# lucasjinreal/yolov7_d2

Measured on AMD Instinct MI355X. Metric: images/sec training, YOLOX-s 640x640 bs=16/GPU, higher is better.
Workload: dtype bf16; 1 GPU; YOLOX-s CSPDarknet+PAFPN 640x640 bs=16/GPU: fwd + SimOTA loss + bwd + grad all-reduce + SGD(momentum) step, uint8 image batch + labels resident in HBM; global_batch=16, parallelism=dp1, hipgraph=True

## Files before the change

### yolov7_d2_amd/csrc/misc_ops.hip

```cpp
#include <stdlib.h>
#include "common.h"

static int ew_blocks(int64_t total, int cap = 4096) {
  int64_t b = (total + 255) / 256;
  if (b > cap) b = cap;
  if (b < 1) b = 1;
  return (int)b;
}

__global__ __launch_bounds__(256) void focus_pack_kernel(const float* __restrict__ img, int N, int H, int W,
                                                         __bf16* out, int ldo) {
  const int Ho = H / 2, Wo = W / 2;
  const int64_t total = (int64_t)N * Ho * Wo;
  for (int64_t idx = blockIdx.x * 256LL + threadIdx.x; idx < total; idx += (int64_t)gridDim.x * 256) {
    const int ox = (int)(idx % Wo);
    const int64_t r = idx / Wo;
    const int oy = (int)(r % Ho), n = (int)(r / Ho);
    float f[16];
#pragma unroll
    for (int q = 0; q < 4; ++q) {
      const int dy = q & 1, dx = q >> 1;
#pragma unroll
      for (int c = 0; c < 3; ++c)
        f[q * 3 + c] = img[(((int64_t)n * 3 + c) * H + (2 * oy + dy)) * W + 2 * ox + dx];
// ... 297 lines not shown
extern "C" int mi_maxpool3x3s2_fwd(const void* x, int ldx, void* y, int ldy, int N, int H, int W, int C, mi_stream_t st) {
  MI_REQUIRE(x && y && C % 8 == 0 && ldx % 8 == 0 && ldy % 8 == 0 && N > 0 && H > 0 && W > 0, "maxpool3x3s2_fwd: args");
  const int64_t total = (int64_t)N * ((H + 1) / 2) * ((W + 1) / 2) * (C / 8);
  hipLaunchKernelGGL(maxpool3x3s2_fwd_kernel, dim3(ew_blocks(total)), dim3(256), 0, (hipStream_t)st, (const __bf16*)x,
                     ldx, (__bf16*)y, ldy, N, H, W, C / 8);
  MI_CHECK_LAUNCH("maxpool3x3s2_fwd");
  return MI_OK;
}
extern "C" int mi_maxpool3x3s2_bwd(const void* x, int ldx, const void* dy, int lddy, void* dx, int lddx, int accumulate,
                                   int N, int H, int W, int C, mi_stream_t st) {
  MI_REQUIRE(x && dy && dx && C % 8 == 0 && ldx % 8 == 0 && lddy % 8 == 0 && lddx % 8 == 0, "maxpool3x3s2_bwd: args");
  const int64_t total = (int64_t)N * H * W * (C / 8);
  hipLaunchKernelGGL(maxpool3x3s2_bwd_kernel, dim3(ew_blocks(total)), dim3(256), 0, (hipStream_t)st, (const __bf16*)x,
                     ldx, (const __bf16*)dy, lddy, (__bf16*)dx, lddx, accumulate, N, H, W, C / 8);
  MI_CHECK_LAUNCH("maxpool3x3s2_bwd");
  return MI_OK;
}

__global__ __launch_bounds__(256) void upsample2x_fwd_kernel(const __bf16* __restrict__ x, int ldx, __bf16* y, int ldy,
                                                             int N, int H, int W, int C8) {
  const int Ho = 2 * H, Wo = 2 * W;
  const int64_t total = (int64_t)N * Ho * Wo * C8;
  for (int64_t idx = blockIdx.x * 256LL + threadIdx.x; idx < total; idx += (int64_t)gridDim.x * 256) {
    const int c8 = (int)(idx % C8);
    int64_t r = idx / C8;
    const int ox = (int)(r % Wo); r /= Wo;
    const int oy = (int)(r % Ho);
    const int n = (int)(r / Ho);
    const bf16x8 v = *(const bf16x8*)(x + (((int64_t)n * H + oy / 2) * W + ox / 2) * ldx + c8 * 8);
    *(bf16x8*)(y + (((int64_t)n * Ho + oy) * Wo + ox) * ldy + c8 * 8) = v;
  }
}
__global__ __launch_bounds__(256) void upsample2x_bwd_kernel(const __bf16* __restrict__ dy, int lddy, __bf16* dx,
                                                             int lddx, int accumulate, int N, int H, int W, int C8) {
  const int Ho = 2 * H, Wo = 2 * W;
  const int64_t total = (int64_t)N * H * W * C8;
  for (int64_t idx = blockIdx.x * 256LL + threadIdx.x; idx < total; idx += (int64_t)gridDim.x * 256) {
    const int c8 = (int)(idx % C8);
    int64_t r = idx / C8;
    const int ix = (int)(r % W); r /= W;
    const int iy = (int)(r % H);
    const int n = (int)(r / H);
    float acc[8];
#pragma unroll
    for (int e = 0; e < 8; ++e) acc[e] = 0.f;
#pragma unroll
    for (int a = 0; a < 2; ++a)
#pragma unroll
      for (int b = 0; b < 2; ++b) {
        const bf16x8 v = *(const bf16x8*)(dy + (((int64_t)n * Ho + 2 * iy + a) * Wo + 2 * ix + b) * lddy + c8 * 8);
#pragma unroll
        for (int e = 0; e < 8; ++e) acc[e] += (float)v[e];
      }
    __bf16* dp = dx + (((int64_t)n * H + iy) * W + ix) * lddx + c8 * 8;
    if (accumulate) {
      const bf16x8 o = *(const bf16x8*)dp;
#pragma unroll
      for (int e = 0; e < 8; ++e) acc[e] += (float)o[e];
    }
    *(bf16x8*)dp = pack8(acc);
  }
}

extern "C" int mi_upsample2x_fwd(const void* x, int ldx, void* y, int ldy, int N, int H, int W, int C,
                                 mi_stream_t st) {
  MI_REQUIRE(x && y && C % 8 == 0 && ldx % 8 == 0 && ldy % 8 == 0, "upsample_fwd: args");
  const int64_t total = (int64_t)N * 4 * H * W * (C / 8);
  hipLaunchKernelGGL(upsample2x_fwd_kernel, dim3(ew_blocks(total)), dim3(256), 0, (hipStream_t)st, (const __bf16*)x,
                     ldx, (__bf16*)y, ldy, N, H, W, C / 8);
  MI_CHECK_LAUNCH("upsample_fwd");
  return MI_OK;
}
extern "C" int mi_upsample2x_bwd(const void* dy, int lddy, void* dx, int lddx, int accumulate, int N, int H, int W,
                                 int C, mi_stream_t st) {
  MI_REQUIRE(dy && dx && C % 8 == 0 && lddy % 8 == 0 && lddx % 8 == 0, "upsample_bwd: args");
  const int64_t total = (int64_t)N * H * W * (C / 8);
  hipLaunchKernelGGL(upsample2x_bwd_kernel, dim3(ew_blocks(total)), dim3(256), 0, (hipStream_t)st, (const __bf16*)dy,
                     lddy, (__bf16*)dx, lddx, accumulate, N, H, W, C / 8);
  MI_CHECK_LAUNCH("upsample_bwd");
  return MI_OK;
}

#define SPP_T 512
__global__ __launch_bounds__(SPP_T) void spp_fwd_plane_kernel(const __bf16* __restrict__ x, int ldx, __bf16* y5,
                                                            __bf16* y9, __bf16* y13, int ldy, uint8_t* idx, int N,
                                                            int H, int W, int C8) {
  extern __shared__ __attribute__((aligned(16))) char smem[];
  const int HW = H * W, C = C8 * 8;
  bf16x8* Xp = (bf16x8*)smem;
  bf16x8* Hv = Xp + HW;
  uint64_t* Hc = (uint64_t*)(Hv + HW);
  const int lb = (gridDim.x % 8 == 0) ? (int)(blockIdx.x % 8) * (int)(gridDim.x / 8) + (int)(blockIdx.x / 8) : (int)blockIdx.x;
  const int c8 = lb % C8, n = lb / C8;
  const int64_t npix = (int64_t)N * HW;
  const __bf16* xb = x + ((int64_t)n * HW) * ldx + c8 * 8;
  for (int p = threadIdx.x; p < HW; p += SPP_T) Xp[p] = *(const bf16x8*)(xb + (int64_t)p * ldx);
  __syncthreads();
  const int k = blockIdx.y, r = 2 + 2 * k;
  for (int p = threadIdx.x; p < HW; p += SPP_T) {
    const int py = p / W, px = p - py * W;
    float m[8];
    uint8_t am[8];
#pragma unroll
    for (int e = 0; e < 8; ++e) { m[e] = -INFINITY; am[e] = 6; }
    for (int dx = -r; dx <= r; ++dx) {
      const int xx = px + dx;
      if (xx < 0 || xx >= W) continue;
      const bf16x8 v = Xp[py * W + xx];
#pragma unroll
      for (int e = 0; e < 8; ++e) {
        const float f = (float)v[e];
        if (f > m[e]) { m[e] = f; am[e] = (uint8_t)(dx + 6); }
      }
    }
    Hv[p] = pack8(m);
    uint64_t pk = 0;
#pragma unroll
    for (int e = 0; e < 8; ++e) pk |= (uint64_t)am[e] << (8 * e);
    Hc[p] = pk;
    *(uint64_t*)(idx + ((int64_t)(3 + k) * npix + (int64_t)n * HW + p) * C + c8 * 8) = pk;
  }
  __syncthreads();
  __bf16* yk = k == 0 ? y5 : (k == 1 ? y9 : y13);
  for (int p = threadIdx.x; p < HW; p += SPP_T) {
    const int py = p / W, px = p - py * W;
    float m[8];
    uint8_t am[8];
#pragma unroll
    for (int e = 0; e < 8; ++e) { m[e] = -INFINITY; am[e] = 6; }
    for (int dy = -r; dy <= r; ++dy) {
      const int yy = py + dy;
      if (yy < 0 || yy >= H) continue;
      const bf16x8 v = Hv[yy * W + px];
#pragma unroll
      for (int e = 0; e < 8; ++e) {
        const float f = (float)v[e];
        if (f > m[e]) { m[e] = f; am[e] = (uint8_t)(dy + 6); }
      }
    }
    const int64_t pix = (int64_t)n * HW + p;
    *(bf16x8*)(yk + pix * ldy + c8 * 8) = pack8(m);
    uint64_t pk = 0;
#pragma unroll
    for (int e = 0; e < 8; ++e) pk |= (uint64_t)am[e] << (8 * e);
    *(uint64_t*)(idx + ((int64_t)k * npix + pix) * C + c8 * 8) = pk;
  }
}

__global__ __launch_bounds__(SPP_T) void spp_bwd_plane_kernel(const __bf16* __restrict__ d5, const __bf16* __restrict__ d9,
                                                            const __bf16* __restrict__ d13, int lddy,
                                                            const uint8_t* __restrict__ idx, __bf16* dx, int lddx,
                                                            int accumulate, int N, int H, int W, int C8) {
  extern __shared__ __attribute__((aligned(16))) char smem[];
  const int HW = H * W, C = C8 * 8;
  bf16x8* Gp = (bf16x8*)smem;
  uint64_t* Dy = (uint64_t*)(Gp + HW);
  uint64_t* Dx = Dy + HW;
  float* Gh = (float*)(Dx + HW);
  const int lb = (gridDim.x % 8 == 0) ? (int)(blockIdx.x % 8) * (int)(gridDim.x / 8) + (int)(blockIdx.x / 8) : (int)blockIdx.x;
  const int c8 = lb % C8, n = lb / C8;
  const int64_t npix = (int64_t)N * HW;
  float acc[2][8];
  for (int i = 0; i < 2; ++i)
#pragma unroll
    for (int e = 0; e < 8; ++e) acc[i][e] = 0.f;
  for (int k = 0; k < 3; ++k) {
    const int r = 2 + 2 * k;
    const __bf16* dk = k == 0 ? d5 : (k == 1 ? d9 : d13);
    __syncthreads();
    for (int p = threadIdx.x; p < HW; p += SPP_T) {
      const int64_t pix = (int64_t)n * HW + p;
      Gp[p] = *(const bf16x8*)(dk + pix * lddy + c8 * 8);
      Dy[p] = *(const uint64_t*)(idx + ((int64_t)k * npix + pix) * C + c8 * 8);
      Dx[p] = *(const uint64_t*)(idx + ((int64_t)(3 + k) * npix + pix) * C + c8 * 8);
    }
    __syncthreads();
    for (int q = threadIdx.x; q < HW; q += SPP_T) {
      const int qy = q / W, qx = q - qy * W;
      float g[8];
#pragma unroll
      for (int e = 0; e < 8; ++e) g[e] = 0.f;
      for (int dy = -r; dy <= r; ++dy) {
        const int oy = qy - dy;
        if (oy < 0 || oy >= H) continue;
        const int o = oy * W + qx;
        const uint64_t pk = Dy[o];
        const bf16x8 gv = Gp[o];
        const uint8_t code = (uint8_t)(dy + 6);
#pragma unroll
        for (int e = 0; e < 8; ++e)
          if ((uint8_t)(pk >> (8 * e)) == code) g[e] += (float)gv[e];
      }
#pragma unroll
      for (int e = 0; e < 8; ++e) Gh[q * 8 + e] = g[e];
    }
    __syncthreads();
#pragma unroll
    for (int i = 0; i < 2; ++i) {
      const int p = threadIdx.x + i * SPP_T;
      if (p >= HW) continue;
      const int py = p / W, px = p - py * W;
      for (int dxx = -r; dxx <= r; ++dxx) {
        const int qx = px - dxx;
        if (qx < 0 || qx >= W) continue;
        const int q = py * W + qx;
        const uint64_t pk = Dx[q];
        const uint8_t code = (uint8_t)(dxx + 6);
#pragma unroll
        for (int e = 0; e < 8; ++e)
          if ((uint8_t)(pk >> (8 * e)) == code) acc[i][e] += Gh[q * 8 + e];
      }
    }
  }
#pragma unroll
  for (int i = 0; i < 2; ++i) {
    const int p = threadIdx.x + i * SPP_T;
    if (p >= HW) continue;
    __bf16* op_ = dx + ((int64_t)n * HW + p) * lddx + c8 * 8;
    float o[8];
#pragma unroll
    for (int e = 0; e < 8; ++e) o[e] = acc[i][e];
    if (accumulate) {
      const bf16x8 ov = *(const bf16x8*)op_;
#pragma unroll
      for (int e = 0; e < 8; ++e) o[e] += (float)ov[e];
    }
    *(bf16x8*)op_ = pack8(o);
  }
}

extern "C" int mi_spp_pool_fwd(const void* x, int ldx, void* y5, void* y9, void* y13, int ldy, uint8_t* idx, int N,
                               int H, int W, int C, mi_stream_t st) {
  MI_REQUIRE(x && y5 && y9 && y13 && idx && C % 8 == 0 && ldx % 8 == 0 && ldy % 8 == 0, "spp_fwd: args");
  const size_t lds = (size_t)H * W * 40;
  MI_REQUIRE(lds <= 160 * 1024, "spp_fwd: plane %dx%d too large for the LDS kernel", H, W);
  static bool attr_done = false;
  if (!attr_done) {
    hipFuncSetAttribute((const void*)spp_fwd_plane_kernel, hipFuncAttributeMaxDynamicSharedMemorySize, 160 * 1024);
    hipFuncSetAttribute((const void*)spp_bwd_plane_kernel, hipFuncAttributeMaxDynamicSharedMemorySize, 160 * 1024);
    attr_done = true;
  }
  hipLaunchKernelGGL(spp_fwd_plane_kernel, dim3(N * (C / 8), 3), dim3(SPP_T), lds, (hipStream_t)st, (const __bf16*)x, ldx,
                     (__bf16*)y5, (__bf16*)y9, (__bf16*)y13, ldy, idx, N, H, W, C / 8);
  MI_CHECK_LAUNCH("spp_fwd");
  return MI_OK;
}
extern "C" int mi_spp_pool_bwd(const void* dy5, const void* dy9, const void* dy13, int lddy, const uint8_t* idx,
                               void* dx, int lddx, int accumulate, int N, int H, int W, int C, mi_stream_t st) {
  MI_REQUIRE(dy5 && dy9 && dy13 && idx && dx && C % 8 == 0 && lddy % 8 == 0 && lddx % 8 == 0, "spp_bwd: args");
  MI_REQUIRE(H * W <= 2 * SPP_T, "spp_bwd: plane %dx%d > %d pixels (register accumulators)", H, W, 2 * SPP_T);
  const size_t lds = (size_t)H * W * 64;
  static bool attr_done = false;
  if (!attr_done) {
    hipFuncSetAttribute((const void*)spp_fwd_plane_kernel, hipFuncAttributeMaxDynamicSharedMemorySize, 160 * 1024);
    hipFuncSetAttribute((const void*)spp_bwd_plane_kernel, hipFuncAttributeMaxDynamicSharedMemorySize, 160 * 1024);
    attr_done = true;
  }
  hipLaunchKernelGGL(spp_bwd_plane_kernel, dim3(N * (C / 8)), dim3(SPP_T), lds, (hipStream_t)st, (const __bf16*)dy5,
                     (const __bf16*)dy9, (const __bf16*)dy13, lddy, idx, (__bf16*)dx, lddx, accumulate, N, H, W, C / 8);
  MI_CHECK_LAUNCH("spp_bwd");
  return MI_OK;
}

__global__ __launch_bounds__(256) void copy_bf16_kernel(const __bf16* __restrict__ src, int lds_, __bf16* dst, int ldd,
                                                        int accumulate, int64_t npix, int C8) {
  const int64_t total = npix * C8;
  for (int64_t idx = blockIdx.x * 256LL + threadIdx.x; idx < total; idx += (int64_t)gridDim.x * 256) {
    const int64_t pix = idx / C8;
    const int c8 = (int)(idx - pix * C8);
    const bf16x8 v = *(const bf16x8*)(src + pix * lds_ + c8 * 8);
    __bf16* dp = dst + pix * ldd + c8 * 8;
    if (accumulate) {
      const bf16x8 o = *(const bf16x8*)dp;
      float f[8];
#pragma unroll
      for (int e = 0; e < 8; ++e) f[e] = (float)o[e] + (float)v[e];
      *(bf16x8*)dp = pack8(f);
    } else {
      *(bf16x8*)dp = v;
    }
  }
}
extern "C" int mi_copy_bf16(const void* src, int lds_, void* dst, int ldd, int accumulate, int64_t npix, int C,
                            mi_stream_t st) {
  MI_REQUIRE(src && dst && C % 8 == 0 && lds_ % 8 == 0 && ldd % 8 == 0, "copy_bf16: args");
  hipLaunchKernelGGL(copy_bf16_kernel, dim3(ew_blocks(npix * (C / 8))), dim3(256), 0, (hipStream_t)st,
                     (const __bf16*)src, lds_, (__bf16*)dst, ldd, accumulate, npix, C / 8);
  MI_CHECK_LAUNCH("copy_bf16");
  return MI_OK;
}

__global__ __launch_bounds__(256) void colsum_stage1_kernel(const __bf16* __restrict__ x, int ldx, int64_t npix,
                                                            int C8N, float* __restrict__ part) {
  __shared__ float red[256 * 8];
  const int tid = threadIdx.x;
  const int c8 = tid % C8N, pl = tid / C8N, PL = 256 / C8N;
  float s[8];
#pragma unroll
  for (int e = 0; e < 8; ++e) s[e] = 0.f;
  if (pl < PL)
    for (int64_t p = (int64_t)blockIdx.x * PL + pl; p < npix; p += (int64_t)gridDim.x * PL) {
      const bf16x8 v = *(const bf16x8*)(x + p * ldx + c8 * 8);
#pragma unroll
      for (int e = 0; e < 8; ++e) s[e] += (float)v[e];
    }
#pragma unroll
  for (int e = 0; e < 8; ++e) red[tid * 8 + e] = (pl < PL) ? s[e] : 0.f;
  __syncthreads();
  const int C = C8N * 8;
  if (tid < C) {
    const int cc8 = tid >> 3, e = tid & 7;
    float a = 0.f;
    for (int q = 0; q < PL; ++q) a += red[(q * C8N + cc8) * 8 + e];
    part[(size_t)blockIdx.x * C + tid] = a;
  }
}
__global__ __launch_bounds__(128) void colsum_stage2_kernel(const float* __restrict__ part, int nblk, int CP, int C,
                                                            float* out, int accumulate) {
  const int c = threadIdx.x;
  if (c >= C) return;
  float a = 0.f;
  for (int b = 0; b < nblk; ++b) a += part[(size_t)b * CP + c];
  out[c] = accumulate ? out[c] + a : a;
}
extern "C" int mi_colsum_bf16(const void* x, int ldx, int64_t npix, int C, float* out, int accumulate, float* ws,
                              mi_stream_t st) {
  MI_REQUIRE(x && out && ws && C > 0 && C <= 128, "colsum: C %d (<=128)", C);
  const int CP = (C + 7) / 8 * 8;
  const int C8N = CP / 8;
  MI_REQUIRE(ldx % 8 == 0 && ((uintptr_t)x % 16) == 0 && ldx >= CP, "colsum: alignment / ld");
  hipStream_t s = (hipStream_t)st;
  const int PL = 256 / C8N;
  int nblk = (int)((npix + PL * 8 - 1) / (PL * 8));
  if (nblk > 128) nblk = 128;
  if (nblk < 1) nblk = 1;
  hipLaunchKernelGGL(colsum_stage1_kernel, dim3(nblk), dim3(256), 0, s, (const __bf16*)x, ldx, npix, C8N, ws);
  MI_CHECK_LAUNCH("colsum1");
  hipLaunchKernelGGL(colsum_stage2_kernel, dim3(1), dim3(128), 0, s, ws, nblk, CP, C, out, accumulate);
  MI_CHECK_LAUNCH("colsum2");
  return MI_OK;
}

// ... 196 lines not shown
```

Measured before the change: 3081 images/sec.

## Compute SPP pools with packed value/position keys and cascaded separable max windows

The SPP forward now packs each bf16 value with its window position into an order-preserving 32-bit key. It then computes the 5/9/13 max pools as a cascade of separable 5-wide passes (SPPF-style) in one block per plane, where before there were three independent direct-window launches. Argmax codes come from the key's position bits. The backward keeps gradients as fp32 in LDS, prefetches the next pool's gradients and codes into registers while the current pool computes, and uses branchless masked adds. This cuts redundant window comparisons and load latency, at the cost of more LDS per pixel and a fallback path for large planes.

```diff
diff --git a/yolov7_d2_amd/csrc/misc_ops.hip b/yolov7_d2_amd/csrc/misc_ops.hip
--- a/yolov7_d2_amd/csrc/misc_ops.hip
+++ b/yolov7_d2_amd/csrc/misc_ops.hip
@@ -403,9 +403,135 @@
 }
 
 #define SPP_T 512
+#define SPP_FWD_LDS_PER_PIXEL 160
+__device__ __forceinline__ uint32_t spp_key(uint32_t b, uint32_t pos8) {
+  const uint32_t nz = b == 0x8000u;
+  const uint32_t img = nz ? 0x8000u : ((b & 0x8000u) ? (~b & 0xFFFFu) : (b | 0x8000u));
+  return (img - 0x80u <= 0xFF00u) ? (img << 16 | pos8 | nz) : 0u;
+}
+__device__ __forceinline__ uint32_t spp_key_bits(uint32_t key) {
+  const uint32_t img = key >> 16;
+  const uint32_t b = (key & 1u) ? 0x8000u : ((img & 0x8000u) ? (img & 0x7FFFu) : (~img & 0xFFFFu));
+  return img ? b : 0xFF80u;
+}
+struct SppK8 { uint32_t v[8]; };
+__device__ __forceinline__ SppK8 spp_ld(const uint4* m, int HW, int p) {
+  const uint4 a = m[p], b = m[HW + p];
+  return SppK8{{a.x, a.y, a.z, a.w, b.x, b.y, b.z, b.w}};
+}
+__device__ __forceinline__ void spp_st(uint4* m, int HW, int p, const SppK8& k) {
+  m[p] = make_uint4(k.v[0], k.v[1], k.v[2], k.v[3]);
+  m[HW + p] = make_uint4(k.v[4], k.v[5], k.v[6], k.v[7]);
+}
+__device__ __forceinline__ SppK8 spp_max(const SppK8& a, const SppK8& b) {
+  SppK8 r;
+#pragma unroll
+  for (int e = 0; e < 8; ++e) r.v[e] = max(a.v[e], b.v[e]);
+  return r;
+}
+__device__ __forceinline__ SppK8 spp_win5(const uint4* m, int HW, int base, int stride, int c, int n) {
+  SppK8 r = spp_ld(m, HW, base + c * stride);
+#pragma unroll
+  for (int d = -2; d <= 2; ++d)
+    if (d) r = spp_max(r, spp_ld(m, HW, base + min(max(c + d, 0), n - 1) * stride));
+  return r;
+}
+__device__ __forceinline__ SppK8 spp_win9(const uint4* m, int HW, int base, int stride, int c, int n) {
+  return spp_max(spp_ld(m, HW, base + max(c - 2, 0) * stride), spp_ld(m, HW, base + min(c + 2, n - 1) * stride));
+}
+__device__ __forceinline__ SppK8 spp_win13(const uint4* m, int HW, int base, int stride, int c, int n) {
+  return spp_max(spp_ld(m, HW, base + c * stride), spp_max(spp_ld(m, HW, base + max(c - 4, 0) * stride),
+                                                           spp_ld(m, HW, base + min(c + 4, n - 1) * stride)));
+}
+__device__ __forceinline__ uint64_t spp_codes(const SppK8& k, uint32_t cb) {
+  uint64_t pk = 0;
+#pragma unroll
+  for (int e = 0; e < 8; ++e) pk |= (uint64_t)((k.v[e] >> 16) ? cb - ((k.v[e] >> 8) & 0xFFu) : 6u) << (8 * e);
+  return pk;
+}
+__device__ __forceinline__ uint4 spp_values(const SppK8& k) {
+  uint32_t w[4];
+#pragma unroll
+  for (int e = 0; e < 4; ++e) w[e] = spp_key_bits(k.v[2 * e]) | spp_key_bits(k.v[2 * e + 1]) << 16;
+  return make_uint4(w[0], w[1], w[2], w[3]);
+}
+__device__ __forceinline__ SppK8 spp_rekey(const SppK8& k, uint32_t pos8) {
+  SppK8 r;
+#pragma unroll
+  for (int e = 0; e < 8; ++e) r.v[e] = (k.v[e] >> 16) ? ((k.v[e] & 0xFFFF0001u) | pos8) : 0u;
+  return r;
+}
 __global__ __launch_bounds__(SPP_T) void spp_fwd_plane_kernel(const __bf16* __restrict__ x, int ldx, __bf16* y5,
                                                             __bf16* y9, __bf16* y13, int ldy, uint8_t* idx, int N,
                                                             int H, int W, int C8) {
+  extern __shared__ __attribute__((aligned(16))) char smem[];
+  const int HW = H * W, C = C8 * 8;
+  uint4* Kx = (uint4*)smem;
+  uint4* H5 = Kx + 2 * HW;
+  uint4* R9 = H5 + 2 * HW;
+  uint4* R13 = R9 + 2 * HW;
+  uint4* T13 = R13 + 2 * HW;
+  const int lb = (gridDim.x % 8 == 0) ? (int)(blockIdx.x % 8) * (int)(gridDim.x / 8) + (int)(blockIdx.x / 8) : (int)blockIdx.x;
+  const int c8 = lb % C8, n = lb / C8;
+  const int64_t npix = (int64_t)N * HW, pix0 = (int64_t)n * HW;
+  const uint16_t* xb = (const uint16_t*)x + pix0 * ldx + c8 * 8;
+  for (int p = threadIdx.x; p < HW; p += SPP_T) {
+    const uint4 v = *(const uint4*)(xb + (int64_t)p * ldx);
+    const uint32_t pos8 = (uint32_t)(255 - p % W) << 8;
+    const uint32_t w[4] = {v.x, v.y, v.z, v.w};
+    SppK8 k;
+#pragma unroll
+    for (int e = 0; e < 4; ++e) {
+      k.v[2 * e] = spp_key(w[e] & 0xFFFFu, pos8);
+      k.v[2 * e + 1] = spp_key(w[e] >> 16, pos8);
+    }
+    spp_st(Kx, HW, p, k);
+  }
+  __syncthreads();
+  uint8_t* cx = idx + (3 * npix + pix0) * C + c8 * 8;
+  uint8_t* cy = idx + pix0 * C + c8 * 8;
+  for (int p = threadIdx.x; p < HW; p += SPP_T) {
+    const int py = p / W, px = p - py * W;
+    const SppK8 h = spp_win5(Kx, HW, py * W, 1, px, W);
+    spp_st(H5, HW, p, h);
+    *(uint64_t*)(cx + (int64_t)p * C) = spp_codes(h, 261u - px);
+  }
+  __syncthreads();
+  for (int p = threadIdx.x; p < HW; p += SPP_T) {
+    const int py = p / W, px = p - py * W;
+    const uint32_t row8 = (uint32_t)(255 - py) << 8;
+    spp_st(Kx, HW, p, spp_rekey(spp_ld(H5, HW, p), row8));
+    const SppK8 h9 = spp_win9(H5, HW, py * W, 1, px, W);
+    *(uint64_t*)(cx + (npix + p) * C) = spp_codes(h9, 261u - px);
+    spp_st(R9, HW, p, spp_rekey(h9, row8));
+    const SppK8 h13 = spp_win13(H5, HW, py * W, 1, px, W);
+    *(uint64_t*)(cx + (2 * npix + p) * C) = spp_codes(h13, 261u - px);
+    spp_st(R13, HW, p, spp_rekey(h13, row8));
+  }
+  __syncthreads();
+  for (int p = threadIdx.x; p < HW; p += SPP_T) {
+    const int py = p / W, px = p - py * W;
+    const SppK8 v = spp_win5(Kx, HW, px, W, py, H);
+    *(uint4*)(y5 + (pix0 + p) * ldy + c8 * 8) = spp_values(v);
+    *(uint64_t*)(cy + (int64_t)p * C) = spp_codes(v, 261u - py);
+    spp_st(H5, HW, p, spp_win5(R9, HW, px, W, py, H));
+    spp_st(T13, HW, p, spp_win5(R13, HW, px, W, py, H));
+  }
+  __syncthreads();
+  for (int p = threadIdx.x; p < HW; p += SPP_T) {
+    const int py = p / W, px = p - py * W;
+    const SppK8 v9 = spp_win9(H5, HW, px, W, py, H);
+    *(uint4*)(y9 + (pix0 + p) * ldy + c8 * 8) = spp_values(v9);
+    *(uint64_t*)(cy + (npix + p) * C) = spp_codes(v9, 261u - py);
+    const SppK8 v13 = spp_win13(T13, HW, px, W, py, H);
+    *(uint4*)(y13 + (pix0 + p) * ldy + c8 * 8) = spp_values(v13);
+    *(uint64_t*)(cy + (2 * npix + p) * C) = spp_codes(v13, 261u - py);
+  }
+}
+
+static __global__ __launch_bounds__(SPP_T) void spp_fwd_taps_kernel(const __bf16* __restrict__ x, int ldx, __bf16* y5,
+                                                                  __bf16* y9, __bf16* y13, int ldy, uint8_t* idx,
+                                                                  int N, int H, int W, int C8) {
   extern __shared__ __attribute__((aligned(16))) char smem[];
   const int HW = H * W, C = C8 * 8;
   bf16x8* Xp = (bf16x8*)smem;
@@ -468,16 +594,22 @@
   }
 }
 
+__device__ __forceinline__ void spp_add_where(float* acc, uint2 codes, uint32_t code, const float4& a, const float4& b) {
+  const float g[8] = {a.x, a.y, a.z, a.w, b.x, b.y, b.z, b.w};
+#pragma unroll
+  for (int e = 0; e < 8; ++e)
+    acc[e] += (((e < 4 ? codes.x : codes.y) >> (8 * (e & 3))) & 0xFFu) == code ? g[e] : 0.f;
+}
 __global__ __launch_bounds__(SPP_T) void spp_bwd_plane_kernel(const __bf16* __restrict__ d5, const __bf16* __restrict__ d9,
                                                             const __bf16* __restrict__ d13, int lddy,
                                                             const uint8_t* __restrict__ idx, __bf16* dx, int lddx,
                                                             int accumulate, int N, int H, int W, int C8) {
   extern __shared__ __attribute__((aligned(16))) char smem[];
   const int HW = H * W, C = C8 * 8;
-  bf16x8* Gp = (bf16x8*)smem;
-  uint64_t* Dy = (uint64_t*)(Gp + HW);
-  uint64_t* Dx = Dy + HW;
-  float* Gh = (float*)(Dx + HW);
+  float4* Gp = (float4*)smem;
+  float4* Gh = Gp + 2 * HW;
+  uint2* Dy = (uint2*)(Gh + 2 * HW);
+  uint2* Dx = Dy + HW;
   const int lb = (gridDim.x % 8 == 0) ? (int)(blockIdx.x % 8) * (int)(gridDim.x / 8) + (int)(blockIdx.x / 8) : (int)blockIdx.x;
   const int c8 = lb % C8, n = lb / C8;
   const int64_t npix = (int64_t)N * HW;
@@ -485,35 +617,49 @@
   for (int i = 0; i < 2; ++i)
 #pragma unroll
     for (int e = 0; e < 8; ++e) acc[i][e] = 0.f;
+  uint4 ng[2];
+  uint2 ny[2], nx[2];
+  auto fetch = [&](int k) {
+    const __bf16* dk = k == 0 ? d5 : (k == 1 ? d9 : d13);
+#pragma unroll
+    for (int i = 0; i < 2; ++i) {
+      const int p = threadIdx.x + i * SPP_T;
+      if (p >= HW) continue;
+      const int64_t pix = (int64_t)n * HW + p;
+      ng[i] = *(const uint4*)(dk + pix * lddy + c8 * 8);
+      ny[i] = *(const uint2*)(idx + ((int64_t)k * npix + pix) * C + c8 * 8);
+      nx[i] = *(const uint2*)(idx + ((int64_t)(3 + k) * npix + pix) * C + c8 * 8);
+    }
+  };
+  fetch(0);
   for (int k = 0; k < 3; ++k) {
     const int r = 2 + 2 * k;
-    const __bf16* dk = k == 0 ? d5 : (k == 1 ? d9 : d13);
     __syncthreads();
-    for (int p = threadIdx.x; p < HW; p += SPP_T) {
-      const int64_t pix = (int64_t)n * HW + p;
-      Gp[p] = *(const bf16x8*)(dk + pix * lddy + c8 * 8);
-      Dy[p] = *(const uint64_t*)(idx + ((int64_t)k * npix + pix) * C + c8 * 8);
-      Dx[p] = *(const uint64_t*)(idx + ((int64_t)(3 + k) * npix + pix) * C + c8 * 8);
+#pragma unroll
+    for (int i = 0; i < 2; ++i) {
+      const int p = threadIdx.x + i * SPP_T;
+      if (p >= HW) continue;
+      Gp[p] = make_float4(__uint_as_float(ng[i].x << 16), __uint_as_float(ng[i].x & 0xFFFF0000u),
+                          __uint_as_float(ng[i].y << 16), __uint_as_float(ng[i].y & 0xFFFF0000u));
+      Gp[HW + p] = make_float4(__uint_as_float(ng[i].z << 16), __uint_as_float(ng[i].z & 0xFFFF0000u),
+                               __uint_as_float(ng[i].w << 16), __uint_as_float(ng[i].w & 0xFFFF0000u));
+      Dy[p] = ny[i];
+      Dx[p] = nx[i];
     }
     __syncthreads();
+    if (k < 2) fetch(k + 1);
     for (int q = threadIdx.x; q < HW; q += SPP_T) {
       const int qy = q / W, qx = q - qy * W;
       float g[8];
 #pragma unroll
       for (int e = 0; e < 8; ++e) g[e] = 0.f;
-      for (int dy = -r; dy <= r; ++dy) {
-        const int oy = qy - dy;
-        if (oy < 0 || oy >= H) continue;
+      const int o1 = max(qy - r, 0);
+      for (int oy = min(qy + r, H - 1); oy >= o1; --oy) {
         const int o = oy * W + qx;
-        const uint64_t pk = Dy[o];
-        const bf16x8 gv = Gp[o];
-        const uint8_t code = (uint8_t)(dy + 6);
-#pragma unroll
-        for (int e = 0; e < 8; ++e)
-          if ((uint8_t)(pk >> (8 * e)) == code) g[e] += (float)gv[e];
+        spp_add_where(g, Dy[o], (uint32_t)(qy - oy + 6), Gp[o], Gp[HW + o]);
       }
-#pragma unroll
-      for (int e = 0; e < 8; ++e) Gh[q * 8 + e] = g[e];
+      Gh[q] = make_float4(g[0], g[1], g[2], g[3]);
+      Gh[HW + q] = make_float4(g[4], g[5], g[6], g[7]);
     }
     __syncthreads();
 #pragma unroll
@@ -521,15 +667,10 @@
       const int p = threadIdx.x + i * SPP_T;
       if (p >= HW) continue;
       const int py = p / W, px = p - py * W;
-      for (int dxx = -r; dxx <= r; ++dxx) {
-        const int qx = px - dxx;
-        if (qx < 0 || qx >= W) continue;
+      const int q1 = max(px - r, 0);
+      for (int qx = min(px + r, W - 1); qx >= q1; --qx) {
         const int q = py * W + qx;
-        const uint64_t pk = Dx[q];
-        const uint8_t code = (uint8_t)(dxx + 6);
-#pragma unroll
-        for (int e = 0; e < 8; ++e)
-          if ((uint8_t)(pk >> (8 * e)) == code) acc[i][e] += Gh[q * 8 + e];
+        spp_add_where(acc[i], Dx[q], (uint32_t)(px - qx + 6), Gh[q], Gh[HW + q]);
       }
     }
   }
@@ -553,16 +694,22 @@
 extern "C" int mi_spp_pool_fwd(const void* x, int ldx, void* y5, void* y9, void* y13, int ldy, uint8_t* idx, int N,
                                int H, int W, int C, mi_stream_t st) {
   MI_REQUIRE(x && y5 && y9 && y13 && idx && C % 8 == 0 && ldx % 8 == 0 && ldy % 8 == 0, "spp_fwd: args");
-  const size_t lds = (size_t)H * W * 40;
-  MI_REQUIRE(lds <= 160 * 1024, "spp_fwd: plane %dx%d too large for the LDS kernel", H, W);
   static bool attr_done = false;
   if (!attr_done) {
     hipFuncSetAttribute((const void*)spp_fwd_plane_kernel, hipFuncAttributeMaxDynamicSharedMemorySize, 160 * 1024);
-    hipFuncSetAttribute((const void*)spp_bwd_plane_kernel, hipFuncAttributeMaxDynamicSharedMemorySize, 160 * 1024);
+    hipFuncSetAttribute((const void*)spp_fwd_taps_kernel, hipFuncAttributeMaxDynamicSharedMemorySize, 160 * 1024);
     attr_done = true;
   }
-  hipLaunchKernelGGL(spp_fwd_plane_kernel, dim3(N * (C / 8), 3), dim3(SPP_T), lds, (hipStream_t)st, (const __bf16*)x, ldx,
-                     (__bf16*)y5, (__bf16*)y9, (__bf16*)y13, ldy, idx, N, H, W, C / 8);
+  const size_t lds = (size_t)H * W * SPP_FWD_LDS_PER_PIXEL;
+  if (lds <= 160 * 1024 && H <= 256 && W <= 256) {
+    hipLaunchKernelGGL(spp_fwd_plane_kernel, dim3(N * (C / 8)), dim3(SPP_T), lds, (hipStream_t)st, (const __bf16*)x, ldx,
+                       (__bf16*)y5, (__bf16*)y9, (__bf16*)y13, ldy, idx, N, H, W, C / 8);
+  } else {
+    const size_t lds_taps = (size_t)H * W * 40;
+    MI_REQUIRE(lds_taps <= 160 * 1024, "spp_fwd: plane %dx%d too large for the LDS kernel", H, W);
+    hipLaunchKernelGGL(spp_fwd_taps_kernel, dim3(N * (C / 8), 3), dim3(SPP_T), lds_taps, (hipStream_t)st, (const __bf16*)x,
+                       ldx, (__bf16*)y5, (__bf16*)y9, (__bf16*)y13, ldy, idx, N, H, W, C / 8);
+  }
   MI_CHECK_LAUNCH("spp_fwd");
   return MI_OK;
 }
@@ -570,10 +717,9 @@
                                void* dx, int lddx, int accumulate, int N, int H, int W, int C, mi_stream_t st) {
   MI_REQUIRE(dy5 && dy9 && dy13 && idx && dx && C % 8 == 0 && lddy % 8 == 0 && lddx % 8 == 0, "spp_bwd: args");
   MI_REQUIRE(H * W <= 2 * SPP_T, "spp_bwd: plane %dx%d > %d pixels (register accumulators)", H, W, 2 * SPP_T);
-  const size_t lds = (size_t)H * W * 64;
+  const size_t lds = (size_t)H * W * 80;
   static bool attr_done = false;
   if (!attr_done) {
-    hipFuncSetAttribute((const void*)spp_fwd_plane_kernel, hipFuncAttributeMaxDynamicSharedMemorySize, 160 * 1024);
     hipFuncSetAttribute((const void*)spp_bwd_plane_kernel, hipFuncAttributeMaxDynamicSharedMemorySize, 160 * 1024);
     attr_done = true;
   }
```

New measurement: 3098 images/sec, median of 6. No clear change (+0.5%).

## Rewrite SPP pooling kernels with packed-key max and fused kernel sizes

Applied to the files above, without the earlier changes.

The SPP forward max-pool kernel now packs each bf16 value together with its coordinate into a sortable 32-bit key, so argmax becomes a plain integer max. Growing windows (5/9/13) are computed incrementally in a single block when the plane fits in one round. Block size is chosen to match the plane size. The backward kernel preloads all three gradients and indices into registers, replaces branches with clamped, predicated taps, and for small planes processes all three kernel sizes in one pass. This cuts redundant LDS scans, divergent branches and kernel work, at the cost of more LDS and registers per block and extra code complexity.

```diff
diff --git a/yolov7_d2_amd/csrc/misc_ops.hip b/yolov7_d2_amd/csrc/misc_ops.hip
--- a/yolov7_d2_amd/csrc/misc_ops.hip
+++ b/yolov7_d2_amd/csrc/misc_ops.hip
@@ -403,139 +403,254 @@
 }
 
 #define SPP_T 512
+__device__ __forceinline__ uint32_t spp_word(uint32_t b, uint32_t cf) {
+  const uint32_t nz = b == 0x8000u ? 1u : 0u;
+  const uint32_t key = nz ? 0x8000u : (b ^ ((b & 0x8000u) ? 0xFFFFu : 0x8000u));
+  return key << 16 | cf | nz;
+}
+__device__ __forceinline__ uint32_t spp_bits(uint32_t w) {
+  const uint32_t key = w >> 16;
+  return key ^ ((key & 0x8000u) ? 0x8000u : 0xFFFFu) ^ ((w & 1u) << 15);
+}
+__device__ __forceinline__ uint32_t spp_coord_field(int c) { return (0x7FFFu - (uint32_t)c) << 1; }
+__device__ __forceinline__ uint2 spp_codes(const uint32_t* m, int c) {
+  const uint32_t c0 = 0x7FFFu + 6u - (uint32_t)c;
+  uint32_t b[8];
+#pragma unroll
+  for (int e = 0; e < 8; ++e) b[e] = c0 - ((m[e] >> 1) & 0x7FFFu);
+  return make_uint2(b[0] | b[1] << 8 | b[2] << 16 | b[3] << 24, b[4] | b[5] << 8 | b[6] << 16 | b[7] << 24);
+}
+template <int R0, int R1>
+__device__ __forceinline__ void spp_scan(const uint4* S, int HW, int base, int stride, int c, int n, uint32_t* m) {
+#pragma unroll
+  for (int d = -R1; d <= R1; ++d) {
+    if (d >= -R0 && d <= R0) continue;
+    const int o = base + min(max(c + d, 0), n - 1) * stride;
+    const uint4 lo = S[o], hi = S[HW + o];
+    m[0] = max(m[0], lo.x); m[1] = max(m[1], lo.y); m[2] = max(m[2], lo.z); m[3] = max(m[3], lo.w);
+    m[4] = max(m[4], hi.x); m[5] = max(m[5], hi.y); m[6] = max(m[6], hi.z); m[7] = max(m[7], hi.w);
+  }
+}
+__device__ __forceinline__ void spp_scan_k(int k, const uint4* S, int HW, int base, int stride, int c, int n, uint32_t* m) {
+#pragma unroll
+  for (int e = 0; e < 8; ++e) m[e] = 0;
+  if (k == 0) spp_scan<-1, 2>(S, HW, base, stride, c, n, m);
+  else if (k == 1) spp_scan<-1, 4>(S, HW, base, stride, c, n, m);
+  else spp_scan<-1, 6>(S, HW, base, stride, c, n, m);
+}
+
+template <int NR, int KG>
 __global__ __launch_bounds__(SPP_T) void spp_fwd_plane_kernel(const __bf16* __restrict__ x, int ldx, __bf16* y5,
                                                             __bf16* y9, __bf16* y13, int ldy, uint8_t* idx, int N,
-                                                            int H, int W, int C8) {
+                                                            int H, int W, int C8, int inplace) {
   extern __shared__ __attribute__((aligned(16))) char smem[];
-  const int HW = H * W, C = C8 * 8;
-  bf16x8* Xp = (bf16x8*)smem;
-  bf16x8* Hv = Xp + HW;
-  uint64_t* Hc = (uint64_t*)(Hv + HW);
+  const int HW = H * W, C = C8 * 8, T = blockDim.x;
+  uint4* Xw = (uint4*)smem;
+  uint4* Hw = inplace ? Xw : Xw + 2 * HW;
   const int lb = (gridDim.x % 8 == 0) ? (int)(blockIdx.x % 8) * (int)(gridDim.x / 8) + (int)(blockIdx.x / 8) : (int)blockIdx.x;
   const int c8 = lb % C8, n = lb / C8;
   const int64_t npix = (int64_t)N * HW;
   const __bf16* xb = x + ((int64_t)n * HW) * ldx + c8 * 8;
-  for (int p = threadIdx.x; p < HW; p += SPP_T) Xp[p] = *(const bf16x8*)(xb + (int64_t)p * ldx);
+  for (int p = threadIdx.x; p < HW; p += T) {
+    const uint4 v = *(const uint4*)(xb + (int64_t)p * ldx);
+    const uint32_t cf = spp_coord_field(p % W);
+    Xw[p] = make_uint4(spp_word(v.x & 0xFFFFu, cf), spp_word(v.x >> 16, cf), spp_word(v.y & 0xFFFFu, cf), spp_word(v.y >> 16, cf));
+    Xw[HW + p] = make_uint4(spp_word(v.z & 0xFFFFu, cf), spp_word(v.z >> 16, cf), spp_word(v.w & 0xFFFFu, cf), spp_word(v.w >> 16, cf));
+  }
   __syncthreads();
-  const int k = blockIdx.y, r = 2 + 2 * k;
-  for (int p = threadIdx.x; p < HW; p += SPP_T) {
+  const int k0 = blockIdx.y * KG;
+  uint32_t h[NR][KG][8];
+#pragma unroll
+  for (int i = 0; i < NR; ++i) {
+    const int p = threadIdx.x + i * T;
+    if (p < HW) {
+      const int py = p / W, px = p - py * W;
+      if constexpr (KG == 3) {
+        uint32_t m[8];
+#pragma unroll
+        for (int e = 0; e < 8; ++e) m[e] = 0;
+        spp_scan<-1, 2>(Xw, HW, py * W, 1, px, W, m);
+#pragma unroll
+        for (int e = 0; e < 8; ++e) h[i][0][e] = m[e];
+        spp_scan<2, 4>(Xw, HW, py * W, 1, px, W, m);
+#pragma unroll
+        for (int e = 0; e < 8; ++e) h[i][1][e] = m[e];
+        spp_scan<4, 6>(Xw, HW, py * W, 1, px, W, m);
+#pragma unroll
+        for (int e = 0; e < 8; ++e) h[i][2][e] = m[e];
+      } else {
+        spp_scan_k(k0, Xw, HW, py * W, 1, px, W, h[i][0]);
+      }
+      const uint32_t cf = spp_coord_field(py);
+#pragma unroll
+      for (int j = 0; j < KG; ++j) {
+        *(uint2*)(idx + ((int64_t)(3 + k0 + j) * npix + (int64_t)n * HW + p) * C + c8 * 8) = spp_codes(h[i][j], px);
+#pragma unroll
+        for (int e = 0; e < 8; ++e) h[i][j][e] = (h[i][j][e] & 0xFFFF0001u) | cf;
+      }
+    }
+  }
+  if (inplace) __syncthreads();
+#pragma unroll
+  for (int i = 0; i < NR; ++i) {
+    const int p = threadIdx.x + i * T;
+    if (p < HW) {
+#pragma unroll
+      for (int j = 0; j < KG; ++j) {
+        Hw[j * 2 * HW + p] = make_uint4(h[i][j][0], h[i][j][1], h[i][j][2], h[i][j][3]);
+        Hw[(j * 2 + 1) * HW + p] = make_uint4(h[i][j][4], h[i][j][5], h[i][j][6], h[i][j][7]);
+      }
+    }
+  }
+  __syncthreads();
+#pragma unroll
+  for (int i = 0; i < NR; ++i) {
+    const int p = threadIdx.x + i * T;
+    if (p < HW) {
+      const int py = p / W, px = p - py * W;
+      const int64_t pix = (int64_t)n * HW + p;
+#pragma unroll
+      for (int j = 0; j < KG; ++j) {
+        const int k = k0 + j;
+        uint32_t m[8];
+        spp_scan_k(k, Hw + j * 2 * HW, HW, px, W, py, H, m);
+        *(uint2*)(idx + ((int64_t)k * npix + pix) * C + c8 * 8) = spp_codes(m, py);
+        __bf16* yk = k == 0 ? y5 : (k == 1 ? y9 : y13);
+        *(uint4*)(yk + pix * ldy + c8 * 8) =
+            make_uint4(spp_bits(m[0]) | spp_bits(m[1]) << 16, spp_bits(m[2]) | spp_bits(m[3]) << 16,
+                       spp_bits(m[4]) | spp_bits(m[5]) << 16, spp_bits(m[6]) | spp_bits(m[7]) << 16);
+      }
+    }
+  }
+}
+
+__device__ __forceinline__ void spp_tap(float* a, uint64_t pk8, uint32_t code, const float* v) {
+  const uint2 pk = make_uint2((uint32_t)pk8, (uint32_t)(pk8 >> 32));
+#pragma unroll
+  for (int e = 0; e < 4; ++e) {
+    a[e] += ((pk.x >> (8 * e)) & 0xFFu) == code ? v[e] : 0.f;
+    a[4 + e] += ((pk.y >> (8 * e)) & 0xFFu) == code ? v[4 + e] : 0.f;
+  }
+}
+template <int R>
+__device__ __forceinline__ void spp_gather_rows(const uint4* G, const uint64_t* Dy, int H, int W, int qy, int qx, float* g) {
+#pragma unroll
+  for (int dy = -R; dy <= R; ++dy) {
+    const int oy = qy - dy;
+    const uint32_t code = (unsigned)oy < (unsigned)H ? (uint32_t)(dy + 6) : 0xFFu;
+    const int o = min(max(oy, 0), H - 1) * W + qx;
+    const uint4 gv = G[o];
+    const float v[8] = {__uint_as_float(gv.x << 16), __uint_as_float(gv.x & 0xFFFF0000u),
+                        __uint_as_float(gv.y << 16), __uint_as_float(gv.y & 0xFFFF0000u),
+                        __uint_as_float(gv.z << 16), __uint_as_float(gv.z & 0xFFFF0000u),
+                        __uint_as_float(gv.w << 16), __uint_as_float(gv.w & 0xFFFF0000u)};
+    spp_tap(g, Dy[o], code, v);
+  }
+}
+template <int R>
+__device__ __forceinline__ void spp_gather_cols(const float4* Gh, int HW, const uint64_t* Dx, int W, int py, int px, float* a) {
+#pragma unroll
+  for (int dxx = -R; dxx <= R; ++dxx) {
+    const int qx = px - dxx;
+    const uint32_t code = (unsigned)qx < (unsigned)W ? (uint32_t)(dxx + 6) : 0xFFu;
+    const int q = py * W + min(max(qx, 0), W - 1);
+    const float4 lo = Gh[q], hi = Gh[HW + q];
+    const float v[8] = {lo.x, lo.y, lo.z, lo.w, hi.x, hi.y, hi.z, hi.w};
+    spp_tap(a, Dx[q], code, v);
+  }
+}
+
+template <int NI>
+__device__ __forceinline__ void spp_bwd_rows(int k, const uint4* G, const uint64_t* Dy, float4* Gh, int HW, int H, int W, int T) {
+#pragma unroll
+  for (int i = 0; i < NI; ++i) {
+    const int q = threadIdx.x + i * T;
+    if (q >= HW) continue;
+    const int qy = q / W, qx = q - qy * W;
+    float g[8];
+#pragma unroll
+    for (int e = 0; e < 8; ++e) g[e] = 0.f;
+    if (k == 0) spp_gather_rows<2>(G, Dy, H, W, qy, qx, g);
+    else if (k == 1) spp_gather_rows<4>(G, Dy, H, W, qy, qx, g);
+    else spp_gather_rows<6>(G, Dy, H, W, qy, qx, g);
+    Gh[q] = make_float4(g[0], g[1], g[2], g[3]);
+    Gh[HW + q] = make_float4(g[4], g[5], g[6], g[7]);
+  }
+}
+template <int NI>
+__device__ __forceinline__ void spp_bwd_cols(int k, const float4* Gh, const uint64_t* Dx, int HW, int W, int T, float (*acc)[8]) {
+#pragma unroll
+  for (int i = 0; i < NI; ++i) {
+    const int p = threadIdx.x + i * T;
+    if (p >= HW) continue;
     const int py = p / W, px = p - py * W;
-    float m[8];
-    uint8_t am[8];
-#pragma unroll
-    for (int e = 0; e < 8; ++e) { m[e] = -INFINITY; am[e] = 6; }
-    for (int dx = -r; dx <= r; ++dx) {
-      const int xx = px + dx;
-      if (xx < 0 || xx >= W) continue;
-      const bf16x8 v = Xp[py * W + xx];
-#pragma unroll
-      for (int e = 0; e < 8; ++e) {
-        const float f = (float)v[e];
-        if (f > m[e]) { m[e] = f; am[e] = (uint8_t)(dx + 6); }
-      }
-    }
-    Hv[p] = pack8(m);
-    uint64_t pk = 0;
-#pragma unroll
-    for (int e = 0; e < 8; ++e) pk |= (uint64_t)am[e] << (8 * e);
-    Hc[p] = pk;
-    *(uint64_t*)(idx + ((int64_t)(3 + k) * npix + (int64_t)n * HW + p) * C + c8 * 8) = pk;
-  }
-  __syncthreads();
-  __bf16* yk = k == 0 ? y5 : (k == 1 ? y9 : y13);
-  for (int p = threadIdx.x; p < HW; p += SPP_T) {
-    const int py = p / W, px = p - py * W;
-    float m[8];
-    uint8_t am[8];
-#pragma unroll
-    for (int e = 0; e < 8; ++e) { m[e] = -INFINITY; am[e] = 6; }
-    for (int dy = -r; dy <= r; ++dy) {
-      const int yy = py + dy;
-      if (yy < 0 || yy >= H) continue;
-      const bf16x8 v = Hv[yy * W + px];
-#pragma unroll
-      for (int e = 0; e < 8; ++e) {
-        const float f = (float)v[e];
-        if (f > m[e]) { m[e] = f; am[e] = (uint8_t)(dy + 6); }
-      }
-    }
-    const int64_t pix = (int64_t)n * HW + p;
-    *(bf16x8*)(yk + pix * ldy + c8 * 8) = pack8(m);
-    uint64_t pk = 0;
-#pragma unroll
-    for (int e = 0; e < 8; ++e) pk |= (uint64_t)am[e] << (8 * e);
-    *(uint64_t*)(idx + ((int64_t)k * npix + pix) * C + c8 * 8) = pk;
-  }
-}
-
+    if (k == 0) spp_gather_cols<2>(Gh, HW, Dx, W, py, px, acc[i]);
+    else if (k == 1) spp_gather_cols<4>(Gh, HW, Dx, W, py, px, acc[i]);
+    else spp_gather_cols<6>(Gh, HW, Dx, W, py, px, acc[i]);
+  }
+}
+
+template <int NI, int KG>
 __global__ __launch_bounds__(SPP_T) void spp_bwd_plane_kernel(const __bf16* __restrict__ d5, const __bf16* __restrict__ d9,
                                                             const __bf16* __restrict__ d13, int lddy,
                                                             const uint8_t* __restrict__ idx, __bf16* dx, int lddx,
                                                             int accumulate, int N, int H, int W, int C8) {
   extern __shared__ __attribute__((aligned(16))) char smem[];
-  const int HW = H * W, C = C8 * 8;
-  bf16x8* Gp = (bf16x8*)smem;
-  uint64_t* Dy = (uint64_t*)(Gp + HW);
-  uint64_t* Dx = Dy + HW;
-  float* Gh = (float*)(Dx + HW);
+  const int HW = H * W, C = C8 * 8, T = blockDim.x;
+  uint4* Gp = (uint4*)smem;
+  float4* Gh = (float4*)(Gp + KG * HW);
+  uint64_t* Dy = (uint64_t*)(Gh + KG * 2 * HW);
+  uint64_t* Dx = Dy + KG * HW;
   const int lb = (gridDim.x % 8 == 0) ? (int)(blockIdx.x % 8) * (int)(gridDim.x / 8) + (int)(blockIdx.x / 8) : (int)blockIdx.x;
   const int c8 = lb % C8, n = lb / C8;
   const int64_t npix = (int64_t)N * HW;
-  float acc[2][8];
-  for (int i = 0; i < 2; ++i)
+  bf16x8 rg[3][NI];
+  uint64_t ry[3][NI], rx[3][NI];
+#pragma unroll
+  for (int k = 0; k < 3; ++k) {
+    const __bf16* dk = k == 0 ? d5 : (k == 1 ? d9 : d13);
+#pragma unroll
+    for (int i = 0; i < NI; ++i) {
+      const int p = threadIdx.x + i * T;
+      if (p >= HW) continue;
+      const int64_t pix = (int64_t)n * HW + p;
+      rg[k][i] = *(const bf16x8*)(dk + pix * lddy + c8 * 8);
+      ry[k][i] = *(const uint64_t*)(idx + ((int64_t)k * npix + pix) * C + c8 * 8);
+      rx[k][i] = *(const uint64_t*)(idx + ((int64_t)(3 + k) * npix + pix) * C + c8 * 8);
+    }
+  }
+  float acc[NI][8];
+#pragma unroll
+  for (int i = 0; i < NI; ++i)
 #pragma unroll
     for (int e = 0; e < 8; ++e) acc[i][e] = 0.f;
+#pragma unroll
   for (int k = 0; k < 3; ++k) {
-    const int r = 2 + 2 * k;
-    const __bf16* dk = k == 0 ? d5 : (k == 1 ? d9 : d13);
+    const int j = KG == 3 ? k : 0;
+    if (KG == 1 && k) __syncthreads();
+#pragma unroll
+    for (int i = 0; i < NI; ++i) {
+      const int p = threadIdx.x + i * T;
+      if (p >= HW) continue;
+      *(bf16x8*)(Gp + j * HW + p) = rg[k][i];
+      Dy[j * HW + p] = ry[k][i];
+      Dx[j * HW + p] = rx[k][i];
+    }
     __syncthreads();
-    for (int p = threadIdx.x; p < HW; p += SPP_T) {
-      const int64_t pix = (int64_t)n * HW + p;
-      Gp[p] = *(const bf16x8*)(dk + pix * lddy + c8 * 8);
-      Dy[p] = *(const uint64_t*)(idx + ((int64_t)k * npix + pix) * C + c8 * 8);
-      Dx[p] = *(const uint64_t*)(idx + ((int64_t)(3 + k) * npix + pix) * C + c8 * 8);
-    }
+    if (KG == 3 && k) spp_bwd_cols<NI>(k - 1, Gh + (k - 1) * 2 * HW, Dx + (k - 1) * HW, HW, W, T, acc);
+    spp_bwd_rows<NI>(k, Gp + j * HW, Dy + j * HW, Gh + j * 2 * HW, HW, H, W, T);
+    if (KG == 1) {
+      __syncthreads();
+      spp_bwd_cols<NI>(k, Gh, Dx, HW, W, T, acc);
+    }
+  }
+  if (KG == 3) {
     __syncthreads();
-    for (int q = threadIdx.x; q < HW; q += SPP_T) {
-      const int qy = q / W, qx = q - qy * W;
-      float g[8];
-#pragma unroll
-      for (int e = 0; e < 8; ++e) g[e] = 0.f;
-      for (int dy = -r; dy <= r; ++dy) {
-        const int oy = qy - dy;
-        if (oy < 0 || oy >= H) continue;
-        const int o = oy * W + qx;
-        const uint64_t pk = Dy[o];
-        const bf16x8 gv = Gp[o];
-        const uint8_t code = (uint8_t)(dy + 6);
-#pragma unroll
-        for (int e = 0; e < 8; ++e)
-          if ((uint8_t)(pk >> (8 * e)) == code) g[e] += (float)gv[e];
-      }
-#pragma unroll
-      for (int e = 0; e < 8; ++e) Gh[q * 8 + e] = g[e];
-    }
-    __syncthreads();
-#pragma unroll
-    for (int i = 0; i < 2; ++i) {
-      const int p = threadIdx.x + i * SPP_T;
-      if (p >= HW) continue;
-      const int py = p / W, px = p - py * W;
-      for (int dxx = -r; dxx <= r; ++dxx) {
-        const int qx = px - dxx;
-        if (qx < 0 || qx >= W) continue;
-        const int q = py * W + qx;
-        const uint64_t pk = Dx[q];
-        const uint8_t code = (uint8_t)(dxx + 6);
-#pragma unroll
-        for (int e = 0; e < 8; ++e)
-          if ((uint8_t)(pk >> (8 * e)) == code) acc[i][e] += Gh[q * 8 + e];
-      }
-    }
-  }
-#pragma unroll
-  for (int i = 0; i < 2; ++i) {
-    const int p = threadIdx.x + i * SPP_T;
+    spp_bwd_cols<NI>(2, Gh + 4 * HW, Dx + 2 * HW, HW, W, T, acc);
+  }
+#pragma unroll
+  for (int i = 0; i < NI; ++i) {
+    const int p = threadIdx.x + i * T;
     if (p >= HW) continue;
     __bf16* op_ = dx + ((int64_t)n * HW + p) * lddx + c8 * 8;
     float o[8];
@@ -550,35 +665,54 @@
   }
 }
 
+static void spp_allow_large_lds() {
+  static bool done = false;
+  if (done) return;
+  const void* ks[] = {(const void*)spp_fwd_plane_kernel<1, 3>, (const void*)spp_fwd_plane_kernel<2, 1>,
+                      (const void*)spp_fwd_plane_kernel<4, 1>, (const void*)spp_fwd_plane_kernel<8, 1>,
+                      (const void*)spp_bwd_plane_kernel<1, 3>, (const void*)spp_bwd_plane_kernel<2, 1>};
+  for (const void* k : ks) hipFuncSetAttribute(k, hipFuncAttributeMaxDynamicSharedMemorySize, 160 * 1024);
+  done = true;
+}
+static int spp_threads(int HW) { return HW >= SPP_T ? SPP_T : (HW + 63) / 64 * 64; }
+
 extern "C" int mi_spp_pool_fwd(const void* x, int ldx, void* y5, void* y9, void* y13, int ldy, uint8_t* idx, int N,
                                int H, int W, int C, mi_stream_t st) {
   MI_REQUIRE(x && y5 && y9 && y13 && idx && C % 8 == 0 && ldx % 8 == 0 && ldy % 8 == 0, "spp_fwd: args");
-  const size_t lds = (size_t)H * W * 40;
-  MI_REQUIRE(lds <= 160 * 1024, "spp_fwd: plane %dx%d too large for the LDS kernel", H, W);
-  static bool attr_done = false;
-  if (!attr_done) {
-    hipFuncSetAttribute((const void*)spp_fwd_plane_kernel, hipFuncAttributeMaxDynamicSharedMemorySize, 160 * 1024);
-    hipFuncSetAttribute((const void*)spp_bwd_plane_kernel, hipFuncAttributeMaxDynamicSharedMemorySize, 160 * 1024);
-    attr_done = true;
-  }
-  hipLaunchKernelGGL(spp_fwd_plane_kernel, dim3(N * (C / 8), 3), dim3(SPP_T), lds, (hipStream_t)st, (const __bf16*)x, ldx,
-                     (__bf16*)y5, (__bf16*)y9, (__bf16*)y13, ldy, idx, N, H, W, C / 8);
+  const int HW = H * W;
+  MI_REQUIRE(HW >= 1 && HW <= 8 * SPP_T, "spp_fwd: plane %dx%d too large for the LDS kernel", H, W);
+  spp_allow_large_lds();
+  const int T = spp_threads(HW), rounds = mi_cdiv(HW, T);
+#define SPP_FWD(NR, KG, lds, inplace)                                                                                    \
+  hipLaunchKernelGGL((spp_fwd_plane_kernel<NR, KG>), dim3(N * (C / 8), 3 / KG), dim3(T), lds, (hipStream_t)st,            \
+                     (const __bf16*)x, ldx, (__bf16*)y5, (__bf16*)y9, (__bf16*)y13, ldy, idx, N, H, W, C / 8, inplace)
+  if (rounds <= 1) {
+    SPP_FWD(1, 3, (size_t)HW * 128, 0);
+  } else {
+    const int inplace = (size_t)HW * 64 > 160 * 1024;
+    const size_t lds = (size_t)HW * (inplace ? 32 : 64);
+    if (rounds <= 2) SPP_FWD(2, 1, lds, inplace);
+    else if (rounds <= 4) SPP_FWD(4, 1, lds, inplace);
+    else SPP_FWD(8, 1, lds, inplace);
+  }
+#undef SPP_FWD
   MI_CHECK_LAUNCH("spp_fwd");
   return MI_OK;
 }
 extern "C" int mi_spp_pool_bwd(const void* dy5, const void* dy9, const void* dy13, int lddy, const uint8_t* idx,
                                void* dx, int lddx, int accumulate, int N, int H, int W, int C, mi_stream_t st) {
   MI_REQUIRE(dy5 && dy9 && dy13 && idx && dx && C % 8 == 0 && lddy % 8 == 0 && lddx % 8 == 0, "spp_bwd: args");
-  MI_REQUIRE(H * W <= 2 * SPP_T, "spp_bwd: plane %dx%d > %d pixels (register accumulators)", H, W, 2 * SPP_T);
-  const size_t lds = (size_t)H * W * 64;
-  static bool attr_done = false;
-  if (!attr_done) {
-    hipFuncSetAttribute((const void*)spp_fwd_plane_kernel, hipFuncAttributeMaxDynamicSharedMemorySize, 160 * 1024);
-    hipFuncSetAttribute((const void*)spp_bwd_plane_kernel, hipFuncAttributeMaxDynamicSharedMemorySize, 160 * 1024);
-    attr_done = true;
-  }
-  hipLaunchKernelGGL(spp_bwd_plane_kernel, dim3(N * (C / 8)), dim3(SPP_T), lds, (hipStream_t)st, (const __bf16*)dy5,
-                     (const __bf16*)dy9, (const __bf16*)dy13, lddy, idx, (__bf16*)dx, lddx, accumulate, N, H, W, C / 8);
+  const int HW = H * W;
+  MI_REQUIRE(HW >= 1 && HW <= 2 * SPP_T, "spp_bwd: plane %dx%d > %d pixels (register accumulators)", H, W, 2 * SPP_T);
+  spp_allow_large_lds();
+  const int T = spp_threads(HW);
+#define SPP_BWD(NI, KG)                                                                                                  \
+  hipLaunchKernelGGL((spp_bwd_plane_kernel<NI, KG>), dim3(N * (C / 8)), dim3(T), (size_t)HW * 64 * KG, (hipStream_t)st,   \
+                     (const __bf16*)dy5, (const __bf16*)dy9, (const __bf16*)dy13, lddy, idx, (__bf16*)dx, lddx, accumulate, \
+                     N, H, W, C / 8)
+  if ((size_t)HW * 64 * 3 <= 80 * 1024) SPP_BWD(1, 3);
+  else SPP_BWD(2, 1);
+#undef SPP_BWD
   MI_CHECK_LAUNCH("spp_bwd");
   return MI_OK;
 }
```

Measured after the change: 3077 images/sec before, 3094 images/sec after (median of 6 runs). No clear change (+0.5%).
